# the3cloud/zktls

Measured on AMD Instinct MI355X. Metric: trace-cells/s, higher is better.
Workload: dtype u32

## Files before the change

zktls_amd/csrc/stark.hip:

```cpp
#include <atomic>

#include "poseidon2.cuh"
#include "kernels.h"
#include "batch.h"

namespace zk {

hipError_t stark_upload_p2_tables(const P2Tables& t, hipStream_t s) { return p2_upload_tables(t, s); }


ZK_D Ext ld_ext(const uint32_t* p) {
    uint4 v = *reinterpret_cast<const uint4*>(p);
    return Ext{{v.x, v.y, v.z, v.w}};
}
ZK_D void st_ext(uint32_t* p, const Ext& e) { *reinterpret_cast<uint4*>(p) = make_uint4(e.c[0], e.c[1], e.c[2], e.c[3]); }

ZK_D Ext group_sum(Ext v, int width) {
    for (int off = width >> 1; off > 0; off >>= 1) {
        Ext o;
        o.c[0] = __shfl_down(v.c[0], off, width);
        o.c[1] = __shfl_down(v.c[1], off, width);
        o.c[2] = __shfl_down(v.c[2], off, width);
        o.c[3] = __shfl_down(v.c[3], off, width);
        v = Ext{{dadd(v.c[0], o.c[0]), dadd(v.c[1], o.c[1]), dadd(v.c[2], o.c[2]), dadd(v.c[3], o.c[3])}};
// ... 36 lines not shown
ZK_D uint4 ld_stream(const uint32_t* p) {
    const u32x4_nt v = __builtin_nontemporal_load(reinterpret_cast<const u32x4_nt*>(p));
    return make_uint4(v.x, v.y, v.z, v.w);
}
ZK_D void dacc1(uint64_t& acc, uint32_t a0, uint32_t b0) {
    const uint64_t t = dmac(a0, b0, acc);
    acc = ((uint64_t)dred((uint32_t)(t >> 32)) << 32) | (uint32_t)t;
}
template <int CTRL>
ZK_D uint32_t dpp_mov(uint32_t v) { return (uint32_t)__builtin_amdgcn_update_dpp(0, (int)v, CTRL, 0xF, 0xF, false); }
ZK_D uint32_t row_group_sum(uint32_t v, int L) {
    if (L > 1) v = dadd(v, dpp_mov<0xB1>(v));
    if (L > 2) v = dadd(v, dpp_mov<0x4E>(v));
    if (L > 4) v = dadd(v, dpp_mov<0x141>(v));
    if (L > 8) v = dadd(v, dpp_mov<0x140>(v));
    return v;
}
__device__ __forceinline__ void logup_addend_kernel_body(const QuotientArgs& a) {
    const int H = a.log_n + 1;
    const uint32_t m = 1u << H;
    const uint32_t p = blockIdx.x * blockDim.x + threadIdx.x;
    if (p >= m) return;
    const uint32_t e = __brev(p) >> (32 - H);
    const uint32_t pn = __brev((e + 2) & (m - 1)) >> (32 - H);
    const uint32_t* row = a.lde + (uint64_t)p * a.ld;
    const uint32_t* prow = a.perm + (uint64_t)p * a.perm_ld;
    const uint32_t* pnrow = a.perm + (uint64_t)pn * a.perm_ld;
    const uint32_t* wl = a.alpha_pow + 16 * (a.width / 4);
    const uint32_t sel_trans = dsub(a.xs[p], a.wn_inv);
    Ext r = ext_zero(), sphi = ext_zero(), sphin = ext_zero();
    for (uint32_t q = 0; q < a.pairs; q++) {
        const uint4 vs = *reinterpret_cast<const uint4*>(row + 8 * q);
        const uint4 vr = *reinterpret_cast<const uint4*>(row + 8 * q + 4);
        const Ext ds = ext_add(ext_add_base(a.gamma, vs.x), ext_mul_base_dev(a.beta, vs.y));
        const Ext dr = ext_add(ext_add_base(a.gamma, vr.x), ext_mul_base_dev(a.beta, vr.y));
        const Ext phi = ld_ext(prow + 4 * q), phin = ld_ext(pnrow + 4 * q);
        const Ext c = ext_sub(ext_mul_dev(ext_mul_dev(phi, ds), dr), ext_sub(dr, ds));
        r = ext_add(r, ext_mul_dev(c, ld_ext(wl + 4 * q)));
        sphi = ext_add(sphi, phi);
        sphin = ext_add(sphin, phin);
    }
    const Ext S = ld_ext(prow + 4 * a.pairs), Sn = ld_ext(pnrow + 4 * a.pairs);
    const Ext F1 = ext_mul_base_dev(ld_ext(wl + 4 * a.pairs), a.sel_first[p]);
    const Ext F2 = ext_mul_base_dev(ld_ext(wl + 4 * (a.pairs + 1)), sel_trans);
    const Ext F3 = ext_mul_base_dev(ld_ext(wl + 4 * (a.pairs + 2)), a.sel_last[p]);
    r = ext_add(r, ext_mul_dev(F1, ext_sub(S, sphi)));
    r = ext_add(r, ext_mul_dev(F2, ext_sub(ext_sub(Sn, S), sphin)));
    r = ext_add(r, ext_mul_dev(F3, ext_sub(S, a.cumsum)));
    st_ext(a.addend_out + 4 * (uint64_t)p, r);
}
__global__ void __launch_bounds__(256) logup_addend_kernel(QuotientArgs a) { logup_addend_kernel_body(a); }
struct logup_addend_kernel_bargs { QuotientArgs a; static logup_addend_kernel_bargs make(QuotientArgs a) { return logup_addend_kernel_bargs{a}; } };
__global__ void __launch_bounds__(256) logup_addend_kernel_batch(const logup_addend_kernel_bargs* __restrict__ zk_arr) { const logup_addend_kernel_bargs& zk_b = zk_arr[blockIdx.z]; logup_addend_kernel_body(zk_b.a); }

hipError_t launch_logup_addend(const QuotientArgs& a, hipStream_t s) {
    const uint64_t m = 2ull << a.log_n;
    ZK_LAUNCH(logup_addend_kernel, logup_addend_kernel_batch, logup_addend_kernel_bargs, dim3((unsigned)((m + 255) / 256)), dim3(256), 0, s, a);
    return hipGetLastError();
}
constexpr int QCHAIN = 16;
template <int NG>
#ifndef QWPE
#define QWPE 2
#endif
__device__ __forceinline__ void quotient_kernel_body(const QuotientArgs& a) {
    const int L = a.lanes_per_row;
    const uint32_t gid = blockIdx.x * blockDim.x + threadIdx.x;
    const int lane = gid % L;
    const int H = a.log_n + 1;
    const uint32_t m = 1u << H;
    const uint32_t nchains = m / QCHAIN;
    const bool live = gid / L < nchains;
    const uint32_t chain = live ? gid / L : 0u;
    const uint32_t parity = chain & 1u;
    uint32_t e = 2u * ((chain >> 1) * QCHAIN) + parity;
    const uint32_t G = a.width / 4;
    const uint32_t inv_zh = parity ? a.inv_zh_odd : a.inv_zh_even;

    uint4 cur[NG], nxt[NG];
    uint32_t p = __brev(e) >> (32 - H);
#pragma unroll
    for (int t = 0; t < NG; t++) {
        const uint32_t g = lane + L * t;
        cur[t] = g < G ? *reinterpret_cast<const uint4*>(a.lde + (uint64_t)p * a.ld + 4 * g) : make_uint4(0, 0, 0, 0);
    }
    constexpr bool HOIST = NG <= 4;
    uint4 W[HOIST ? NG : 1][4];
    if (HOIST) {
#pragma unroll
        for (int t = 0; t < NG; t++) {
            const uint32_t g = lane + L * t;
            const uint4* wp = reinterpret_cast<const uint4*>(a.alpha_pow + 16 * (g < G ? g : 0u));
#pragma unroll
            for (int i = 0; i < 4; i++) W[HOIST ? t : 0][i] = wp[i];
        }
    }
    for (int step = 0; step < QCHAIN; step++) {
        const uint32_t en = (e + 2) & (m - 1);
        const uint32_t pn = __brev(en) >> (32 - H);
#pragma unroll
        for (int t = 0; t < NG; t++) {
            const uint32_t g = lane + L * t;
            nxt[t] = g < G ? ld_stream(a.lde + (uint64_t)pn * a.ld + 4 * g) : make_uint4(0, 0, 0, 0);
        }
        const uint32_t x = a.xs[p];
        const uint32_t sel_first = a.sel_first[p];
        const uint32_t sel_trans = dsub(x, a.wn_inv);
        uint64_t acc[4] = {0, 0, 0, 0};
#pragma unroll
        for (int t = 0; t < NG; t++) {
            const uint32_t g = lane + L * t;
            if (g < G) {
                const uint4 v = cur[t];
                const uint4* wp = reinterpret_cast<const uint4*>(a.alpha_pow + 16 * g);
                const uint4 w0 = HOIST ? W[HOIST ? t : 0][0] : wp[0], w1 = HOIST ? W[HOIST ? t : 0][1] : wp[1];
                const uint4 w2 = HOIST ? W[HOIST ? t : 0][2] : wp[2], kk = HOIST ? W[HOIST ? t : 0][3] : wp[3];
                const uint32_t aab = dmul(dmont_lazy(v.x, v.x), v.y);
                const uint32_t c1 = dsub(dsub(v.z, aab), kk.x);
                const uint32_t ab = dmul(v.x, v.y);
                const uint32_t c2 = dmul(dsub_lazy(dsub(dsub(nxt[t].w, ab), v.z), kk.y), sel_trans);
                const uint32_t c3 = dmul(dsub_lazy(v.w, kk.z), sel_first);
                dacc2(acc[0], w0.x, c1, w1.x, c2); dacc1(acc[0], w2.x, c3);
                dacc2(acc[1], w0.y, c1, w1.y, c2); dacc1(acc[1], w2.y, c3);
                dacc2(acc[2], w0.z, c1, w1.z, c2); dacc1(acc[2], w2.z, c3);
                dacc2(acc[3], w0.w, c1, w1.w, c2); dacc1(acc[3], w2.w, c3);
            }
        }
        Ext r = Ext{{dacc_finish(acc[0]), dacc_finish(acc[1]), dacc_finish(acc[2]), dacc_finish(acc[3])}};
        if (a.addend && lane == 0) r = ext_add(r, ld_ext(a.addend + 4 * (uint64_t)p));
#pragma unroll
        for (int i = 0; i < 4; i++) r.c[i] = row_group_sum(r.c[i], L);
        if (lane == 0 && live) {
            r = ext_mul_base_dev(r, inv_zh);
            st_ext(a.out + ((uint64_t)parity * (m >> 1) + (e >> 1)) * 4, r);
            if (a.lde_out) st_ext(a.lde_out + (uint64_t)p * a.lde_ld + 4u * parity, r);
        }
#pragma unroll
        for (int t = 0; t < NG; t++) cur[t] = nxt[t];
        e = en; p = pn;
    }
}
template <int NG>
#ifndef QWPE
#define QWPE 2
#endif
__global__ void __launch_bounds__(256) __attribute__((amdgpu_waves_per_eu(QWPE, QWPE))) quotient_kernel(QuotientArgs a) { quotient_kernel_body<NG>(a); }
struct quotient_kernel_bargs { QuotientArgs a; static quotient_kernel_bargs make(QuotientArgs a) { return quotient_kernel_bargs{a}; } };
template <int NG>
#ifndef QWPE
#define QWPE 2
#endif
__global__ void __launch_bounds__(256) __attribute__((amdgpu_waves_per_eu(QWPE, QWPE))) quotient_kernel_batch(const quotient_kernel_bargs* __restrict__ zk_arr) { const quotient_kernel_bargs& zk_b = zk_arr[blockIdx.z]; quotient_kernel_body<NG>(zk_b.a); }

hipError_t launch_quotient(const QuotientArgs& a, hipStream_t s) {
    const uint64_t m = 2ull << a.log_n;
    const uint64_t threads = (m / QCHAIN) * a.lanes_per_row;
    const uint32_t G = a.width / 4;
    const int ng = (int)((G + a.lanes_per_row - 1) / a.lanes_per_row);
    const dim3 grid((unsigned)((threads + 255) / 256)), block(256);
    switch (ng) {
        case 1: ZK_LAUNCH(quotient_kernel<1>, quotient_kernel_batch<1>, quotient_kernel_bargs, grid, block, 0, s, a); break;
        case 2: ZK_LAUNCH(quotient_kernel<2>, quotient_kernel_batch<2>, quotient_kernel_bargs, grid, block, 0, s, a); break;
        case 3: ZK_LAUNCH(quotient_kernel<3>, quotient_kernel_batch<3>, quotient_kernel_bargs, grid, block, 0, s, a); break;
        case 4: ZK_LAUNCH(quotient_kernel<4>, quotient_kernel_batch<4>, quotient_kernel_bargs, grid, block, 0, s, a); break;
        case 5: case 6: case 7: case 8: ZK_LAUNCH(quotient_kernel<8>, quotient_kernel_batch<8>, quotient_kernel_bargs, grid, block, 0, s, a); break;
        default: ZK_LAUNCH(quotient_kernel<16>, quotient_kernel_batch<16>, quotient_kernel_bargs, grid, block, 0, s, a); break;
    }
    return hipGetLastError();
}

__device__ __forceinline__ void quotient_air_kernel_body(const QuotientAirArgs& a) {
    const int H = a.log_n + a.log_qd;
    const uint32_t m = 1u << H, nq = 1u << a.log_qd;
    const uint32_t p = blockIdx.x * blockDim.x + threadIdx.x;
    if (p >= m) return;
    const uint32_t e = __brev(p) >> (32 - H);
    const uint32_t pn = __brev((e + nq) & (m - 1)) >> (32 - H);
    const uint32_t* local = a.lde + (uint64_t)p * a.ld;
    const uint32_t* next = a.lde + (uint64_t)pn * a.ld;
    const uint32_t x = a.xs[p];
    const uint32_t sel_first = a.sel_first[p], sel_last = a.sel_last[p], sel_trans = dsub(x, a.wn_inv);
    uint64_t acc[4] = {0, 0, 0, 0};
    const uint32_t* w = a.body;
    for (uint32_t k = 0; k < a.n_constraints; k++) {
        const uint32_t sel = *w++, nt = *w++;
        uint32_t c = 0;
        for (uint32_t t = 0; t < nt; t++) {
            uint32_t prod = *w++;
            const uint32_t d = *w++;
            for (uint32_t j = 0; j < d; j++) {
                const uint32_t v = *w++, kind = v >> 30, idx = v & 0xFFFFu;
                const uint32_t val = kind == 0 ? local[idx] : (kind == 1 ? next[idx] : a.pub[idx]);
                prod = dmul(prod, val);
            }
            c = dadd(c, prod);
        }
        if (sel) c = dmul(c, sel == 1 ? sel_first : (sel == 2 ? sel_last : sel_trans));
        const uint4 wt = *reinterpret_cast<const uint4*>(a.weights + 4 * (uint64_t)k);
        dacc1(acc[0], wt.x, c); dacc1(acc[1], wt.y, c); dacc1(acc[2], wt.z, c); dacc1(acc[3], wt.w, c);
    }
    const uint32_t chunk = e & (nq - 1u);
    Ext r = Ext{{dacc_finish(acc[0]), dacc_finish(acc[1]), dacc_finish(acc[2]), dacc_finish(acc[3])}};
    if (a.addend) r = ext_add(r, ld_ext(a.addend + 4 * (uint64_t)p));
    const uint32_t iz = chunk == 0 ? a.inv_zh[0] : (chunk == 1 ? a.inv_zh[1] : (chunk == 2 ? a.inv_zh[2] : a.inv_zh[3]));
    r = ext_mul_base_dev(r, iz);
    st_ext(a.out + ((uint64_t)chunk * (m >> a.log_qd) + (e >> a.log_qd)) * 4, r);
    if (a.lde_out) st_ext(a.lde_out + (uint64_t)p * a.lde_ld + 4u * chunk, r);
}
__global__ void __launch_bounds__(256) quotient_air_kernel(QuotientAirArgs a) { quotient_air_kernel_body(a); }
struct quotient_air_kernel_bargs { QuotientAirArgs a; static quotient_air_kernel_bargs make(QuotientAirArgs a) { return quotient_air_kernel_bargs{a}; } };
__global__ void __launch_bounds__(256) quotient_air_kernel_batch(const quotient_air_kernel_bargs* __restrict__ zk_arr) { const quotient_air_kernel_bargs& zk_b = zk_arr[blockIdx.z]; quotient_air_kernel_body(zk_b.a); }

__device__ __forceinline__ uint32_t air_group_e0(const QuotientAirArgs& a, uint32_t g) { return ((g >> a.log_qd) * 8u << a.log_qd) + (g & ((1u << a.log_qd) - 1u)); }
__device__ __forceinline__ uint32_t air_row_of(const QuotientAirArgs& a, uint32_t e0, uint32_t r) {
    const int H = a.log_n + a.log_qd;
    return __brev((e0 + (r << a.log_qd)) & ((1u << H) - 1u)) >> (32 - H);
}
__device__ __forceinline__ void air_load8(const uint32_t* slots, uint32_t base, uint32_t (&v)[8]) {
    const uint32_t* b = slots + base;
#pragma unroll
    for (int q = 0; q < 8; q++) v[q] = b[4 * q];
}
template <int NT>
__device__ __forceinline__ void air_stage_extras(const QuotientAirArgs& a, uint32_t* slots, uint32_t e0, uint32_t tid) {
    const uint32_t W4 = a.width >> 2;
    if (tid < 8) {
        const uint32_t p = air_row_of(a, e0, tid);
        const uint4 ex = {a.sel_first[p], a.sel_last[p], dsub(a.xs[p], a.wn_inv), MONTY_R1};
        *reinterpret_cast<uint4*>(slots + AIR_GP * W4 + 4u * tid) = ex;
    }
    for (uint32_t i = tid >> 3; i < a.n_public; i += NT / 8) slots[air_lds_base(2 * a.width + AIR_SLOT_EXTRA + i, a.width) + 4u * (tid & 7u)] = a.pub[i];
}
__device__ __forceinline__ void air_store_point(const QuotientAirArgs& a, uint32_t e, Ext r) {
    const int H = a.log_n + a.log_qd;
    const uint32_t m = 1u << H, nq = 1u << a.log_qd;
    const uint32_t p = __brev(e) >> (32 - H);
    if (a.addend) r = ext_add(r, ld_ext(a.addend + 4 * (uint64_t)p));
    const uint32_t chunk = e & (nq - 1u);
    const uint32_t iz = chunk == 0 ? a.inv_zh[0] : (chunk == 1 ? a.inv_zh[1] : (chunk == 2 ? a.inv_zh[2] : a.inv_zh[3]));
    r = ext_mul_base_dev(r, iz);
    st_ext(a.out + ((uint64_t)chunk * (m >> a.log_qd) + (e >> a.log_qd)) * 4, r);
    if (a.lde_out) st_ext(a.lde_out + (uint64_t)p * a.lde_ld + 4u * chunk, r);
}
template <int NT>
__device__ __forceinline__ void quotient_air_terms_kernel_body(const QuotientAirArgs& a) {
    constexpr int PTS = 8;
    static_assert(NT == 64 || NT == 128 || NT == 256, "one, two or four wavefronts per group");
    extern __shared__ uint32_t slots[];
    const uint32_t tid = threadIdx.x, W4 = a.width >> 2;
    const uint32_t mask = (1u << (a.log_n + a.log_qd)) - 1u;
    const uint32_t e0 = air_group_e0(a, blockIdx.x);
#pragma unroll
    for (int r = 0; r < 9; r++) {
        const uint4* row = reinterpret_cast<const uint4*>(a.lde + (uint64_t)air_row_of(a, e0, r) * a.ld);
        for (uint32_t cg = tid; cg < W4; cg += NT) *reinterpret_cast<uint4*>(slots + AIR_GP * cg + 4u * r) = row[cg];
    }
    air_stage_extras<NT>(a, slots, e0, tid);
    __syncthreads();
    uint64_t acc[PTS][4];
#pragma unroll
    for (int q = 0; q < PTS; q++)
#pragma unroll
        for (int i = 0; i < 4; i++) acc[q][i] = 0;
    const uint4* recs = reinterpret_cast<const uint4*>(a.recs);
    auto load8 = [&](uint32_t o, uint32_t (&v)[PTS]) { air_load8(slots, o, v); };
    auto product = [&](const uint4& o, uint32_t (&prod)[PTS]) {
        const uint32_t n = o.z >> 16;
        uint32_t v[PTS];
        load8(o.x & 0xFFFFu, prod);
        const uint32_t offs[4] = {o.x >> 16, o.y & 0xFFFFu, o.y >> 16, o.z & 0xFFFFu};
        for (uint32_t k = 1; k < n; k++) {
            load8(offs[k - 1], v);
#pragma unroll
            for (int q = 0; q < PTS; q++) prod[q] = dmul(prod[q], v[q]);
        }
    };
    for (uint32_t t = 2 * tid; t < a.n_terms; t += 2 * NT) {
        const uint4 ca = recs[2 * (size_t)t], oa = recs[2 * (size_t)t + 1], cb = recs[2 * (size_t)t + 2], ob = recs[2 * (size_t)t + 3];
        uint32_t pa[PTS], pb[PTS];
        product(oa, pa);
        product(ob, pb);
#pragma unroll
        for (int q = 0; q < PTS; q++) {
            dacc2(acc[q][0], ca.x, pa[q], cb.x, pb[q]); dacc2(acc[q][1], ca.y, pa[q], cb.y, pb[q]);
            dacc2(acc[q][2], ca.z, pa[q], cb.z, pb[q]); dacc2(acc[q][3], ca.w, pa[q], cb.w, pb[q]);
        }
    }
    __syncthreads();
    constexpr int PITCH = NT + 1, SL = NT / 32;
#pragma unroll
    for (int q = 0; q < PTS; q++)
#pragma unroll
        for (int i = 0; i < 4; i++) slots[(size_t)(q * 4 + i) * PITCH + tid] = dacc_finish(acc[q][i]);
    __syncthreads();
    {
        const uint32_t j = tid / SL, sl = tid % SL;
        uint32_t sum = 0;
        for (uint32_t i = sl; i < (uint32_t)NT; i += SL) sum = dadd(sum, slots[(size_t)j * PITCH + i]);
        __syncthreads();
        slots[(size_t)j * PITCH + sl] = sum;
    }
    __syncthreads();
    if (tid < (uint32_t)PTS) {
        Ext r;
        for (int i = 0; i < 4; i++) {
            uint32_t sum = 0;
            for (int k = 0; k < SL; k++) sum = dadd(sum, slots[(size_t)(tid * 4 + i) * PITCH + k]);
            r.c[i] = sum;
// ... 473 lines not shown
        }
#pragma unroll
        for (int k = 0; k < NPTS; k++) {
            Ext w[4];
#pragma unroll
            for (int j = 0; j < 4; j++) w[j] = ld_ext(a.xw + 4 * ((uint64_t)k * a.xw_stride + q[j]));
#pragma unroll
            for (int i = 0; i < 4; i++) {
                dacc2(acc[k][i][0], v[0].x, w[0].c[i], v[1].x, w[1].c[i]); dacc2(acc[k][i][0], v[2].x, w[2].c[i], v[3].x, w[3].c[i]);
                dacc2(acc[k][i][1], v[0].y, w[0].c[i], v[1].y, w[1].c[i]); dacc2(acc[k][i][1], v[2].y, w[2].c[i], v[3].y, w[3].c[i]);
                dacc2(acc[k][i][2], v[0].z, w[0].c[i], v[1].z, w[1].c[i]); dacc2(acc[k][i][2], v[2].z, w[2].c[i], v[3].z, w[3].c[i]);
                dacc2(acc[k][i][3], v[0].w, w[0].c[i], v[1].w, w[1].c[i]); dacc2(acc[k][i][3], v[2].w, w[2].c[i], v[3].w, w[3].c[i]);
            }
        }
    }
#pragma unroll
    for (int k = 0; k < NPTS; k++) {
        uint32_t mine[16];
#pragma unroll
        for (int c = 0; c < 4; c++)
#pragma unroll
            for (int i = 0; i < 4; i++) mine[4 * c + i] = dacc_finish(acc[k][i][c]);
        __syncthreads();
#pragma unroll
        for (int e = 0; e < 16; e++) red[threadIdx.x * 16 + e] = mine[e];
        __syncthreads();
        if (ty == 0 && active) {
            for (int y = 1; y < TY; y++)
#pragma unroll
                for (int e = 0; e < 16; e++) mine[e] = dadd(mine[e], red[(y * TX + tx) * 16 + e]);
            uint4* dst = reinterpret_cast<uint4*>(a.partial + 4 * (((uint64_t)blockIdx.x * NPTS + k) * a.width + col));
#pragma unroll
            for (int c = 0; c < 4; c++) dst[c] = make_uint4(mine[4 * c], mine[4 * c + 1], mine[4 * c + 2], mine[4 * c + 3]);
        }
    }
}
template <int NPTS>
__global__ void __launch_bounds__(256) open_partial4_kernel(OpenArgs a) { open_partial4_kernel_body<NPTS>(a); }
struct open_partial4_kernel_bargs { OpenArgs a; static open_partial4_kernel_bargs make(OpenArgs a) { return open_partial4_kernel_bargs{a}; } };
template <int NPTS>
__global__ void __launch_bounds__(256) open_partial4_kernel_batch(const open_partial4_kernel_bargs* __restrict__ zk_arr) { const open_partial4_kernel_bargs& zk_b = zk_arr[blockIdx.z]; open_partial4_kernel_body<NPTS>(zk_b.a); }

__device__ __forceinline__ void open_final_kernel_body(const uint32_t* partial, uint32_t nchunks, int npts, uint32_t width, const Ext& scale0, const Ext& scale1, uint32_t* out) {
    const uint32_t idx = blockIdx.x;
    const uint32_t k = idx / width, col = idx % width;
    Ext sum = ext_zero();
    for (uint32_t c = threadIdx.x; c < nchunks; c += 64) sum = ext_add(sum, ld_ext(partial + 4 * (((uint64_t)c * npts + k) * width + col)));
    sum = group_sum(sum, 64);
    if (threadIdx.x == 0) st_ext(out + 4 * (uint64_t)idx, ext_neg(ext_mul_dev(sum, k ? scale1 : scale0)));
}
__global__ void __launch_bounds__(64) open_final_kernel(const uint32_t* partial, uint32_t nchunks, int npts, uint32_t width, Ext scale0, Ext scale1, uint32_t* out) { open_final_kernel_body(partial, nchunks, npts, width, scale0, scale1, out); }
struct open_final_kernel_bargs { const uint32_t* partial; uint32_t nchunks; int npts; uint32_t width; Ext scale0; Ext scale1; uint32_t* out; static open_final_kernel_bargs make(const uint32_t* partial, uint32_t nchunks, int npts, uint32_t width, Ext scale0, Ext scale1, uint32_t* out) { return open_final_kernel_bargs{partial, nchunks, npts, width, scale0, scale1, out}; } };
__global__ void __launch_bounds__(64) open_final_kernel_batch(const open_final_kernel_bargs* __restrict__ zk_arr) { const open_final_kernel_bargs& zk_b = zk_arr[blockIdx.z]; open_final_kernel_body(zk_b.partial, zk_b.nchunks, zk_b.npts, zk_b.width, zk_b.scale0, zk_b.scale1, zk_b.out); }

bool open_uses_quads(uint32_t width, uint64_t ld, const uint32_t* mat) {
    return width >= 64 && width % 4 == 0 && ld % 4 == 0 && ((uintptr_t)mat & 15u) == 0;
}
size_t open_chunks(uint64_t rows, uint32_t width, uint64_t ld, const uint32_t* mat) {
    const uint64_t per = open_uses_quads(width, ld, mat) ? OPEN_ROWS4 : OPEN_ROWS;
    return (size_t)((rows + per - 1) / per);
}
hipError_t launch_open(const OpenArgs& a0, int npts, const Ext& scale0, const Ext& scale1, uint32_t* out, hipStream_t s) {
    OpenArgs a = a0;
    const bool quads = open_uses_quads(a.width, a.ld, a.mat);
    const uint32_t nchunks = (uint32_t)open_chunks(a.rows, a.width, a.ld, a.mat);
    if (quads) {
        a.tx = 1;
        while (a.tx < (int)(a.width / 4) && a.tx < 64) a.tx <<= 1;
        dim3 grid(nchunks, (a.width / 4 + a.tx - 1) / a.tx);
        if (npts == 1) ZK_LAUNCH(open_partial4_kernel<1>, open_partial4_kernel_batch<1>, open_partial4_kernel_bargs, grid, dim3(256), 0, s, a);
        else ZK_LAUNCH(open_partial4_kernel<2>, open_partial4_kernel_batch<2>, open_partial4_kernel_bargs, grid, dim3(256), 0, s, a);
    } else {
        dim3 grid(nchunks, (a.width + a.tx - 1) / a.tx);
        if (npts == 1) ZK_LAUNCH(open_partial_kernel<1>, open_partial_kernel_batch<1>, open_partial_kernel_bargs, grid, dim3(256), 0, s, a);
        else ZK_LAUNCH(open_partial_kernel<2>, open_partial_kernel_batch<2>, open_partial_kernel_bargs, grid, dim3(256), 0, s, a);
    }
    hipError_t e = hipGetLastError();
    if (e != hipSuccess) return e;
    const uint32_t n = (uint32_t)npts * a.width;
    ZK_LAUNCH(open_final_kernel, open_final_kernel_batch, open_final_kernel_bargs, dim3(n), dim3(64), 0, s, a.partial, nchunks, npts, a.width, scale0, scale1, out);
    return hipGetLastError();
}

__device__ __forceinline__ void rowdot_kernel_body(const uint32_t* __restrict__ mat, uint64_t ld, uint32_t width, uint64_t rows, int L, const uint32_t* __restrict__ alpha_pow, uint32_t* __restrict__ out_at) {
    const uint64_t gid = (uint64_t)blockIdx.x * blockDim.x + threadIdx.x;
    const uint64_t p = gid / L;
    const int lane = (int)(gid % L);
    if (p >= rows) return;
    const uint32_t* row = mat + p * ld;
    uint64_t acc[4] = {0, 0, 0, 0};
    const uint32_t nq = width / 4;
    for (uint32_t q = lane; q < nq; q += L) {
        const uint4 v = ld_stream(row + 4 * q);
        const uint4* ap = reinterpret_cast<const uint4*>(alpha_pow + 16 * q);
        const uint4 a0 = ap[0], a1 = ap[1], a2 = ap[2], a3 = ap[3];
        dacc2(acc[0], a0.x, v.x, a1.x, v.y); dacc2(acc[0], a2.x, v.z, a3.x, v.w);
        dacc2(acc[1], a0.y, v.x, a1.y, v.y); dacc2(acc[1], a2.y, v.z, a3.y, v.w);
        dacc2(acc[2], a0.z, v.x, a1.z, v.y); dacc2(acc[2], a2.z, v.z, a3.z, v.w);
        dacc2(acc[3], a0.w, v.x, a1.w, v.y); dacc2(acc[3], a2.w, v.z, a3.w, v.w);
    }
    Ext r;
#pragma unroll
    for (int i = 0; i < 4; i++) r.c[i] = row_group_sum(dacc_finish(acc[i]), L);
    if (lane == 0) st_ext(out_at + 4 * p, r);
}
__global__ void __launch_bounds__(256) rowdot_kernel(const uint32_t* __restrict__ mat, uint64_t ld, uint32_t width, uint64_t rows, int L, const uint32_t* __restrict__ alpha_pow, uint32_t* __restrict__ out_at) { rowdot_kernel_body(mat, ld, width, rows, L, alpha_pow, out_at); }
struct rowdot_kernel_bargs { const uint32_t* mat; uint64_t ld; uint32_t width; uint64_t rows; int L; const uint32_t* alpha_pow; uint32_t* out_at; static rowdot_kernel_bargs make(const uint32_t* mat, uint64_t ld, uint32_t width, uint64_t rows, int L, const uint32_t* alpha_pow, uint32_t* out_at) { return rowdot_kernel_bargs{mat, ld, width, rows, L, alpha_pow, out_at}; } };
__global__ void __launch_bounds__(256) rowdot_kernel_batch(const rowdot_kernel_bargs* __restrict__ zk_arr) { const rowdot_kernel_bargs& zk_b = zk_arr[blockIdx.z]; rowdot_kernel_body(zk_b.mat, zk_b.ld, zk_b.width, zk_b.rows, zk_b.L, zk_b.alpha_pow, zk_b.out_at); }

constexpr int ROWDOT_TRIPS = 16;
template <int NK>
__device__ __forceinline__ void rowdot_regs_kernel_body(const uint32_t* __restrict__ mat, uint64_t ld, uint32_t width, uint64_t rows, int L, const uint32_t* __restrict__ alpha_pow, uint32_t* __restrict__ out_at) {
    const int lane = (int)(threadIdx.x % L);
    const uint32_t nq = width / 4;
    const uint64_t rows_per_trip = 256 / L;
    const uint64_t r0 = (uint64_t)blockIdx.x * rows_per_trip * ROWDOT_TRIPS + threadIdx.x / L;
    uint4 a0[NK], a1[NK], a2[NK], a3[NK];
#pragma unroll
    for (int k = 0; k < NK; k++) {
        const uint32_t q = lane + (uint32_t)L * k;
        const uint4* ap = reinterpret_cast<const uint4*>(alpha_pow + 16 * (q < nq ? q : 0));
        a0[k] = ap[0]; a1[k] = ap[1]; a2[k] = ap[2]; a3[k] = ap[3];
    }
    for (int t = 0; t < ROWDOT_TRIPS; t++) {
        const uint64_t p = r0 + (uint64_t)t * rows_per_trip;
        if (p >= rows) return;
        const uint32_t* row = mat + p * ld;
        uint4 v[NK];
#pragma unroll
        for (int k = 0; k < NK; k++) {
            const uint32_t q = lane + (uint32_t)L * k;
            v[k] = q < nq ? ld_stream(row + 4 * q) : make_uint4(0, 0, 0, 0);
        }
        uint64_t acc[4] = {0, 0, 0, 0};
#pragma unroll
        for (int k = 0; k < NK; k++) {
            dacc2(acc[0], a0[k].x, v[k].x, a1[k].x, v[k].y); dacc2(acc[0], a2[k].x, v[k].z, a3[k].x, v[k].w);
            dacc2(acc[1], a0[k].y, v[k].x, a1[k].y, v[k].y); dacc2(acc[1], a2[k].y, v[k].z, a3[k].y, v[k].w);
            dacc2(acc[2], a0[k].z, v[k].x, a1[k].z, v[k].y); dacc2(acc[2], a2[k].z, v[k].z, a3[k].z, v[k].w);
            dacc2(acc[3], a0[k].w, v[k].x, a1[k].w, v[k].y); dacc2(acc[3], a2[k].w, v[k].z, a3[k].w, v[k].w);
        }
        Ext r;
#pragma unroll
        for (int i = 0; i < 4; i++) r.c[i] = row_group_sum(dacc_finish(acc[i]), L);
        if (lane == 0) st_ext(out_at + 4 * p, r);
    }
}
template <int NK>
__global__ void __launch_bounds__(256) rowdot_regs_kernel(const uint32_t* __restrict__ mat, uint64_t ld, uint32_t width, uint64_t rows, int L, const uint32_t* __restrict__ alpha_pow, uint32_t* __restrict__ out_at) { rowdot_regs_kernel_body<NK>(mat, ld, width, rows, L, alpha_pow, out_at); }
struct rowdot_regs_kernel_bargs { const uint32_t* mat; uint64_t ld; uint32_t width; uint64_t rows; int L; const uint32_t* alpha_pow; uint32_t* out_at; static rowdot_regs_kernel_bargs make(const uint32_t* mat, uint64_t ld, uint32_t width, uint64_t rows, int L, const uint32_t* alpha_pow, uint32_t* out_at) { return rowdot_regs_kernel_bargs{mat, ld, width, rows, L, alpha_pow, out_at}; } };
template <int NK>
__global__ void __launch_bounds__(256) rowdot_regs_kernel_batch(const rowdot_regs_kernel_bargs* __restrict__ zk_arr) { const rowdot_regs_kernel_bargs& zk_b = zk_arr[blockIdx.z]; rowdot_regs_kernel_body<NK>(zk_b.mat, zk_b.ld, zk_b.width, zk_b.rows, zk_b.L, zk_b.alpha_pow, zk_b.out_at); }

static hipError_t launch_rowdot(const uint32_t* mat, uint64_t ld, uint32_t width, uint64_t rows, const uint32_t* alpha_pow, uint32_t* out_at, hipStream_t s);
__device__ __forceinline__ void reduced_combine_kernel_body(const ReducedArgs& a, const uint32_t* __restrict__ at_in, const uint32_t* __restrict__ ap_in) {
    const uint64_t p = (uint64_t)blockIdx.x * blockDim.x + threadIdx.x;
    if (p >= a.rows) return;
    const Ext at = ld_ext(at_in + 4 * p);
    const uint4* qrow = reinterpret_cast<const uint4*>(a.qlde + p * a.q_ld);
    Ext aq = ext_zero();
    for (uint32_t h = 0; h < a.q_width / 8; h++) {
        const uint4 q0 = qrow[2 * h], q1 = qrow[2 * h + 1];
        const uint32_t qv[8] = {q0.x, q0.y, q0.z, q0.w, q1.x, q1.y, q1.z, q1.w};
#pragma unroll
        for (int j = 0; j < 8; j++) aq = ext_add(aq, ext_mul_base_dev(ld_ext(a.alpha_pow + 4 * (8 * h + j)), qv[j]));
    }
    const Ext d1 = ld_ext(a.dinv + 4 * p), d2 = ld_ext(a.dinv + 4 * (a.rows + p));
    Ext r = ext_mul_dev(a.off_loc, ext_mul_dev(ext_sub(at, a.y_loc), d1));
    r = ext_add(r, ext_mul_dev(a.off_next, ext_mul_dev(ext_sub(at, a.y_next), d2)));
    if (a.p_width) {
        const Ext ap = ld_ext(ap_in + 4 * p);
        r = ext_add(r, ext_mul_dev(a.off_pl, ext_mul_dev(ext_sub(ap, a.y_pl), d1)));
        r = ext_add(r, ext_mul_dev(a.off_pn, ext_mul_dev(ext_sub(ap, a.y_pn), d2)));
    }
    r = ext_add(r, ext_mul_dev(a.off_q, ext_mul_dev(ext_sub(aq, a.y_q), d1)));
    if (a.accumulate) r = ext_add(r, ld_ext(a.out + 4 * p));
    st_ext(a.out + 4 * p, r);
}
__global__ void __launch_bounds__(256) reduced_combine_kernel(ReducedArgs a, const uint32_t* __restrict__ at_in, const uint32_t* __restrict__ ap_in) { reduced_combine_kernel_body(a, at_in, ap_in); }
struct reduced_combine_kernel_bargs { ReducedArgs a; const uint32_t* at_in; const uint32_t* ap_in; static reduced_combine_kernel_bargs make(ReducedArgs a, const uint32_t* at_in, const uint32_t* ap_in) { return reduced_combine_kernel_bargs{a, at_in, ap_in}; } };
__global__ void __launch_bounds__(256) reduced_combine_kernel_batch(const reduced_combine_kernel_bargs* __restrict__ zk_arr) { const reduced_combine_kernel_bargs& zk_b = zk_arr[blockIdx.z]; reduced_combine_kernel_body(zk_b.a, zk_b.at_in, zk_b.ap_in); }

static int lanes_for(uint32_t width) { int g = (int)(width / 4), l = 1; while (l < g && l < 16) l <<= 1; return l; }
int rowdot_form(uint32_t width, uint64_t rows) {
    const int L = lanes_for(width);
    const uint32_t nq = width / 4;
    const int nk = (int)((nq + L - 1) / L);
    const uint64_t rows_per_wg = (uint64_t)(256 / L) * ROWDOT_TRIPS;
    return (nk >= 1 && nk <= 4 && rows % (256 / L) == 0 && rows >= rows_per_wg) ? nk : 0;
}
static hipError_t launch_rowdot(const uint32_t* mat, uint64_t ld, uint32_t width, uint64_t rows, const uint32_t* alpha_pow, uint32_t* out_at, hipStream_t s) {
    const int L = lanes_for(width);
    const int form = rowdot_form(width, rows);
    if (form) {
        const uint64_t rows_per_wg = (uint64_t)(256 / L) * ROWDOT_TRIPS;
        const dim3 grid((unsigned)((rows + rows_per_wg - 1) / rows_per_wg)), block(256);
        switch (form) {
            case 1: ZK_LAUNCH(rowdot_regs_kernel<1>, rowdot_regs_kernel_batch<1>, rowdot_regs_kernel_bargs, grid, block, 0, s, mat, ld, width, rows, L, alpha_pow, out_at); break;
            case 2: ZK_LAUNCH(rowdot_regs_kernel<2>, rowdot_regs_kernel_batch<2>, rowdot_regs_kernel_bargs, grid, block, 0, s, mat, ld, width, rows, L, alpha_pow, out_at); break;
            case 3: ZK_LAUNCH(rowdot_regs_kernel<3>, rowdot_regs_kernel_batch<3>, rowdot_regs_kernel_bargs, grid, block, 0, s, mat, ld, width, rows, L, alpha_pow, out_at); break;
            default: ZK_LAUNCH(rowdot_regs_kernel<4>, rowdot_regs_kernel_batch<4>, rowdot_regs_kernel_bargs, grid, block, 0, s, mat, ld, width, rows, L, alpha_pow, out_at); break;
        }
        return hipGetLastError();
    }
    const uint64_t threads = rows * L;
    ZK_LAUNCH(rowdot_kernel, rowdot_kernel_batch, rowdot_kernel_bargs, dim3((unsigned)((threads + 255) / 256)), dim3(256), 0, s, mat, ld, width, rows, L, alpha_pow, out_at);
    return hipGetLastError();
}
hipError_t launch_reduced_opening(const ReducedArgs& a, uint32_t* scratch_at, hipStream_t s) {
    hipError_t e = launch_rowdot(a.tlde, a.t_ld, a.width, a.rows, a.alpha_pow, scratch_at, s);
    if (e != hipSuccess) return e;
    uint32_t* scratch_ap = scratch_at + 4 * a.rows;
    if (a.p_width) {
        e = launch_rowdot(a.plde, a.p_ld, a.p_width, a.rows, a.alpha_pow, scratch_ap, s);
        if (e != hipSuccess) return e;
    }
    ZK_LAUNCH(reduced_combine_kernel, reduced_combine_kernel_batch, reduced_combine_kernel_bargs, dim3((unsigned)((a.rows + 255) / 256)), dim3(256), 0, s, a, scratch_at, scratch_ap);
    return hipGetLastError();
}

constexpr int PERM_BLOCK = 256;
__device__ __forceinline__ void perm_rows_kernel_body(const PermArgs& a, uint32_t* __restrict__ block_tot) {
    __shared__ uint32_t sh[PERM_BLOCK * 4];
    const uint64_t i = (uint64_t)blockIdx.x * PERM_BLOCK + threadIdx.x;
    Ext sum = ext_zero();
    if (i < a.rows) {
        const uint32_t* row = a.trace + i * a.ld;
        uint32_t* prow = a.out + i * a.out_ld;
        for (uint32_t q = 0; q < a.pairs; q++) {
            const uint4 vs = *reinterpret_cast<const uint4*>(row + 8 * q);
            const uint4 vr = *reinterpret_cast<const uint4*>(row + 8 * q + 4);
            const Ext ds = ext_add(ext_add_base(a.gamma, vs.x), ext_mul_base_dev(a.beta, vs.y));
            const Ext dr = ext_add(ext_add_base(a.gamma, vr.x), ext_mul_base_dev(a.beta, vr.y));
            const Ext d = ext_mul_dev(ds, dr);
            const Ext phi = ext_eq(d, ext_zero()) ? ext_sub(ext_inv_dev(ds), ext_inv_dev(dr)) : ext_mul_dev(ext_sub(dr, ds), ext_inv_dev(d));
            st_ext(prow + 4 * q, phi);
            sum = ext_add(sum, phi);
        }
    }
    for (int k = 0; k < 4; k++) sh[threadIdx.x * 4 + k] = sum.c[k];
    __syncthreads();
    for (int off = 1; off < PERM_BLOCK; off <<= 1) {
        Ext o = ext_zero();
        if ((int)threadIdx.x >= off) o = Ext{{sh[(threadIdx.x - off) * 4], sh[(threadIdx.x - off) * 4 + 1], sh[(threadIdx.x - off) * 4 + 2], sh[(threadIdx.x - off) * 4 + 3]}};
        __syncthreads();
        sum = ext_add(sum, o);
        for (int k = 0; k < 4; k++) sh[threadIdx.x * 4 + k] = sum.c[k];
        __syncthreads();
    }
    if (i < a.rows) st_ext(a.out + i * a.out_ld + 4 * a.pairs, sum);
    if (threadIdx.x == PERM_BLOCK - 1) st_ext(block_tot + 4 * (uint64_t)blockIdx.x, sum);
}
__global__ void __launch_bounds__(PERM_BLOCK) perm_rows_kernel(PermArgs a, uint32_t* __restrict__ block_tot) { perm_rows_kernel_body(a, block_tot); }
struct perm_rows_kernel_bargs { PermArgs a; uint32_t* block_tot; static perm_rows_kernel_bargs make(PermArgs a, uint32_t* block_tot) { return perm_rows_kernel_bargs{a, block_tot}; } };
__global__ void __launch_bounds__(PERM_BLOCK) perm_rows_kernel_batch(const perm_rows_kernel_bargs* __restrict__ zk_arr) { const perm_rows_kernel_bargs& zk_b = zk_arr[blockIdx.z]; perm_rows_kernel_body(zk_b.a, zk_b.block_tot); }

__device__ __forceinline__ void perm_scan_blocks_kernel_body(uint32_t* block_tot, uint32_t nblocks) {
    __shared__ uint32_t sh[1024 * 4];
    const uint32_t per = (nblocks + 1023) / 1024;
    const uint32_t b0 = threadIdx.x * per;
    Ext sum = ext_zero();
    for (uint32_t k = 0; k < per && b0 + k < nblocks; k++) sum = ext_add(sum, ld_ext(block_tot + 4 * (uint64_t)(b0 + k)));
    for (int k = 0; k < 4; k++) sh[threadIdx.x * 4 + k] = sum.c[k];
    __syncthreads();
    Ext incl = sum;
    for (int off = 1; off < 1024; off <<= 1) {
        Ext o = ext_zero();
        if ((int)threadIdx.x >= off) o = Ext{{sh[(threadIdx.x - off) * 4], sh[(threadIdx.x - off) * 4 + 1], sh[(threadIdx.x - off) * 4 + 2], sh[(threadIdx.x - off) * 4 + 3]}};
        __syncthreads();
        incl = ext_add(incl, o);
        for (int k = 0; k < 4; k++) sh[threadIdx.x * 4 + k] = incl.c[k];
        __syncthreads();
    }
    Ext run = ext_sub(incl, sum);
    for (uint32_t k = 0; k < per && b0 + k < nblocks; k++) {
        const Ext t = ld_ext(block_tot + 4 * (uint64_t)(b0 + k));
        st_ext(block_tot + 4 * (uint64_t)(b0 + k), run);
        run = ext_add(run, t);
    }
}
__global__ void __launch_bounds__(1024) perm_scan_blocks_kernel(uint32_t* block_tot, uint32_t nblocks) { perm_scan_blocks_kernel_body(block_tot, nblocks); }
struct perm_scan_blocks_kernel_bargs { uint32_t* block_tot; uint32_t nblocks; static perm_scan_blocks_kernel_bargs make(uint32_t* block_tot, uint32_t nblocks) { return perm_scan_blocks_kernel_bargs{block_tot, nblocks}; } };
__global__ void __launch_bounds__(1024) perm_scan_blocks_kernel_batch(const perm_scan_blocks_kernel_bargs* __restrict__ zk_arr) { const perm_scan_blocks_kernel_bargs& zk_b = zk_arr[blockIdx.z]; perm_scan_blocks_kernel_body(zk_b.block_tot, zk_b.nblocks); }

__device__ __forceinline__ void perm_fixup_kernel_body(const PermArgs& a, const uint32_t* __restrict__ block_off) {
    const uint64_t i = (uint64_t)blockIdx.x * PERM_BLOCK + threadIdx.x;
    if (i >= a.rows) return;
    uint32_t* sp = a.out + i * a.out_ld + 4 * a.pairs;
    st_ext(sp, ext_add(ld_ext(sp), ld_ext(block_off + 4 * (uint64_t)blockIdx.x)));
}
__global__ void __launch_bounds__(PERM_BLOCK) perm_fixup_kernel(PermArgs a, const uint32_t* __restrict__ block_off) { perm_fixup_kernel_body(a, block_off); }
struct perm_fixup_kernel_bargs { PermArgs a; const uint32_t* block_off; static perm_fixup_kernel_bargs make(PermArgs a, const uint32_t* block_off) { return perm_fixup_kernel_bargs{a, block_off}; } };
__global__ void __launch_bounds__(PERM_BLOCK) perm_fixup_kernel_batch(const perm_fixup_kernel_bargs* __restrict__ zk_arr) { const perm_fixup_kernel_bargs& zk_b = zk_arr[blockIdx.z]; perm_fixup_kernel_body(zk_b.a, zk_b.block_off); }

hipError_t launch_perm_trace(const PermArgs& a, uint32_t* block_scratch, hipStream_t s) {
    const uint32_t nblocks = (uint32_t)((a.rows + PERM_BLOCK - 1) / PERM_BLOCK);
    ZK_LAUNCH(perm_rows_kernel, perm_rows_kernel_batch, perm_rows_kernel_bargs, dim3(nblocks), dim3(PERM_BLOCK), 0, s, a, block_scratch);
    hipError_t e = hipGetLastError();
    if (e != hipSuccess) return e;
    ZK_LAUNCH(perm_scan_blocks_kernel, perm_scan_blocks_kernel_batch, perm_scan_blocks_kernel_bargs, dim3(1), dim3(1024), 0, s, block_scratch, nblocks);
    e = hipGetLastError();
    if (e != hipSuccess) return e;
    ZK_LAUNCH(perm_fixup_kernel, perm_fixup_kernel_batch, perm_fixup_kernel_bargs, dim3(nblocks), dim3(PERM_BLOCK), 0, s, a, block_scratch);
    return hipGetLastError();
}

ZK_D Ext lookup_fingerprint(const LookupArgs& lk, const uint32_t* rec, const uint32_t* row, const uint8_t* cm = nullptr) {
    Ext d = ext_add_base(lk.gamma, rec[2]);
    for (uint32_t v = 0; v < rec[3]; v++) d = ext_add(d, ext_mul_base_dev(lk.bpow[v + 1], row[cm ? cm[rec[4 + v]] : rec[4 + v]]));
    return d;
}
ZK_D uint32_t lookup_mult(const uint32_t* rec, const uint32_t* row, const uint8_t* cm = nullptr) {
    const uint32_t m = rec[1] == 0xFFFFFFFFu ? MONTY_R1 : row[cm ? cm[rec[1]] : rec[1]];
    return rec[0] ? (m ? P - m : 0u) : m;
}
ZK_D const uint32_t* lookup_stage_rows(const LookupArgs& lk, const uint32_t* mat, uint64_t ld, uint64_t row0, uint64_t rows, uint32_t* dyn, const uint8_t** cm_out,
                                       const uint32_t* pre = nullptr, uint64_t pre_ld = 0, uint32_t pre_w = 0) {
    uint8_t* cm = reinterpret_cast<uint8_t*>(dyn);
    uint32_t* tile = dyn + LOOKUP_MAX_COLS / 4;
    const uint32_t pitch = lk.n_used | 1u, tid = threadIdx.x;
    for (uint32_t i = tid; i < LOOKUP_MAX_COLS / 4; i += blockDim.x) dyn[i] = reinterpret_cast<const uint32_t*>(lk.cmap)[i];
    __syncthreads();
    const uint32_t q = tid & 3u;
    for (uint32_t m = lk.chunk_mask; m; m &= m - 1u) {
        const uint32_t col = 16u * (uint32_t)(__ffs((int)m) - 1) + 4u * q;
        const uint8_t k0 = cm[col], k1 = cm[col + 1], k2 = cm[col + 2], k3 = cm[col + 3];
        if ((k0 & k1 & k2 & k3) == 0xFF) continue;
        for (uint32_t r = tid >> 2; r < 256u; r += blockDim.x >> 2) {
            if (row0 + r >= rows) break;
            const bool from_pre = pre != nullptr && col < pre_w;
            const uint32_t* src = from_pre ? pre + (row0 + r) * pre_ld + col : mat + (row0 + r) * ld + (col - (pre ? pre_w : 0u));
            uint32_t* dst = tile + r * pitch;
            if (from_pre || col - (pre ? pre_w : 0u) + 3 < ld) {
                const uint4 v = *reinterpret_cast<const uint4*>(src);
                if (k0 != 0xFF) dst[k0] = v.x;
                if (k1 != 0xFF) dst[k1] = v.y;
                if (k2 != 0xFF) dst[k2] = v.z;
                if (k3 != 0xFF) dst[k3] = v.w;
            } else {
                const uint32_t mc = col - (pre ? pre_w : 0u);
                if (k0 != 0xFF && mc < ld) dst[k0] = src[0];
                if (k1 != 0xFF && mc + 1 < ld) dst[k1] = src[1];
                if (k2 != 0xFF && mc + 2 < ld) dst[k2] = src[2];
            }
        }
    }
// ... 213 lines not shown
```

Baseline: 20.95 billion.

## Add LDS-staged streaming kernels for quotient and row-dot reductions

Adds new quotient and rowdot kernels in which each wave stages 64 rows × 32 columns slices through a padded LDS tile. Loads are coalesced and the next slice is prefetched into registers, so each lane reduces one full row with no cross-lane shuffle reduction. The quotient path also reads the neighbouring row from LDS for the transition constraint. This is meant to cut uncoalesced strided global loads and shuffle overhead, at the cost of LDS use and wave-level fences, and only applies when the width is a multiple of 32 and there are enough rows.

Result: faster. 21.36 billion (median of 6 runs) (+2.0%).

```diff
diff --git a/zktls_amd/csrc/stark.hip b/zktls_amd/csrc/stark.hip
--- a/zktls_amd/csrc/stark.hip
+++ b/zktls_amd/csrc/stark.hip
@@ -212,8 +212,100 @@
 #endif
 __global__ void __launch_bounds__(256) __attribute__((amdgpu_waves_per_eu(QWPE, QWPE))) quotient_kernel_batch(const quotient_kernel_bargs* __restrict__ zk_arr) { const quotient_kernel_bargs& zk_b = zk_arr[blockIdx.z]; quotient_kernel_body<NG>(zk_b.a); }
 
+constexpr int SLICE_COLS = 32;
+constexpr int SLICE_PITCH = SLICE_COLS + 4;
+constexpr uint64_t STREAM_MIN_ROWS = 2048;
+ZK_D void wave_lds_handover() {
+    __builtin_amdgcn_fence(__ATOMIC_RELEASE, "wavefront");
+    __builtin_amdgcn_wave_barrier();
+    __builtin_amdgcn_fence(__ATOMIC_ACQUIRE, "wavefront");
+}
+#ifdef ZKHIP_AB_HOOKS
+static bool stream_forms_off() { const char* e = getenv("ZKHIP_STREAM_OLD"); return e && atoi(e) != 0; }
+#endif
+
+__device__ __forceinline__ void quotient_stream_kernel_body(const QuotientArgs& a) {
+    __shared__ __attribute__((aligned(16))) uint32_t tile[4][65 * SLICE_PITCH];
+    const uint32_t lane = threadIdx.x & 63u, wave = threadIdx.x >> 6;
+    const int H = a.log_n + 1;
+    const uint32_t m = 1u << H;
+    const uint32_t wpp = m >> 7;
+    const uint32_t gw = blockIdx.x * 4u + wave;
+    if (gw >= 2u * wpp) return;
+    const uint32_t parity = gw / wpp, j0 = (gw % wpp) * 64u;
+    uint32_t* t = tile[wave];
+    const uint32_t part = lane & 7u, sub = lane >> 3;
+    const uint32_t* src[9];
+#pragma unroll
+    for (int k = 0; k < 9; k++) {
+        const uint32_t j = j0 + 8u * k + (k < 8 ? sub : 0u);
+        const uint32_t pr = __brev((2u * j + parity) & (m - 1)) >> (32 - H);
+        src[k] = a.lde + (uint64_t)pr * a.ld + 4u * part;
+    }
+    const bool tail = lane < 8u;
+    uint4 pf[9];
+#pragma unroll
+    for (int k = 0; k < 8; k++) pf[k] = ld_stream(src[k]);
+    pf[8] = tail ? ld_stream(src[8]) : make_uint4(0, 0, 0, 0);
+
+    const uint32_t j = j0 + lane;
+    const uint32_t p = __brev(2u * j + parity) >> (32 - H);
+    uint32_t sel_first = a.sel_first[p];
+    const uint32_t sel_trans = dsub(a.xs[p], a.wn_inv);
+    asm("" : "+v"(sel_first));
+    const uint32_t nsl = a.width / SLICE_COLS;
+    uint64_t acc[4] = {0, 0, 0, 0};
+    for (uint32_t s = 0; s < nsl; s++) {
+#pragma unroll
+        for (int k = 0; k < 8; k++) *reinterpret_cast<uint4*>(t + (8u * k + sub) * SLICE_PITCH + 4u * part) = pf[k];
+        if (tail) *reinterpret_cast<uint4*>(t + 64u * SLICE_PITCH + 4u * part) = pf[8];
+        if (s + 1 < nsl) {
+#pragma unroll
+            for (int k = 0; k < 8; k++) pf[k] = ld_stream(src[k] + SLICE_COLS * (s + 1));
+            if (tail) pf[8] = ld_stream(src[8] + SLICE_COLS * (s + 1));
+        }
+        wave_lds_handover();
+        const uint4* wp = reinterpret_cast<const uint4*>(a.alpha_pow + 16u * (SLICE_COLS / 4) * s);
+#pragma unroll
+        for (int g = 0; g < SLICE_COLS / 4; g++) {
+            const uint4 v = *reinterpret_cast<const uint4*>(t + lane * SLICE_PITCH + 4 * g);
+            const uint32_t dn = t[(lane + 1u) * SLICE_PITCH + 4 * g + 3];
+            const uint4 w0 = wp[4 * g], w1 = wp[4 * g + 1], w2 = wp[4 * g + 2], kk = wp[4 * g + 3];
+            const uint32_t aab = dmul(dmont_lazy(v.x, v.x), v.y);
+            const uint32_t c1 = dsub(dsub(v.z, aab), kk.x);
+            const uint32_t ab = dmul(v.x, v.y);
+            const uint32_t c2 = dmul(dsub_lazy(dsub(dsub(dn, ab), v.z), kk.y), sel_trans);
+            const uint32_t c3 = dmul(dsub_lazy(v.w, kk.z), sel_first);
+            dacc2(acc[0], w0.x, c1, w1.x, c2); dacc1(acc[0], w2.x, c3);
+            dacc2(acc[1], w0.y, c1, w1.y, c2); dacc1(acc[1], w2.y, c3);
+            dacc2(acc[2], w0.z, c1, w1.z, c2); dacc1(acc[2], w2.z, c3);
+            dacc2(acc[3], w0.w, c1, w1.w, c2); dacc1(acc[3], w2.w, c3);
+        }
+        wave_lds_handover();
+    }
+    Ext r = Ext{{dacc_finish(acc[0]), dacc_finish(acc[1]), dacc_finish(acc[2]), dacc_finish(acc[3])}};
+    if (a.addend) r = ext_add(r, ld_ext(a.addend + 4 * (uint64_t)p));
+    r = ext_mul_base_dev(r, parity ? a.inv_zh_odd : a.inv_zh_even);
+    st_ext(a.out + ((uint64_t)parity * (m >> 1) + j) * 4, r);
+    if (a.lde_out) st_ext(a.lde_out + (uint64_t)p * a.lde_ld + 4u * parity, r);
+}
+__global__ void __launch_bounds__(256) quotient_stream_kernel(QuotientArgs a) { quotient_stream_kernel_body(a); }
+struct quotient_stream_kernel_bargs { QuotientArgs a; static quotient_stream_kernel_bargs make(QuotientArgs a) { return quotient_stream_kernel_bargs{a}; } };
+__global__ void __launch_bounds__(256) quotient_stream_kernel_batch(const quotient_stream_kernel_bargs* __restrict__ zk_arr) { const quotient_stream_kernel_bargs& zk_b = zk_arr[blockIdx.z]; quotient_stream_kernel_body(zk_b.a); }
+
+static bool quotient_stream_form(const QuotientArgs& a) {
+#ifdef ZKHIP_AB_HOOKS
+    if (stream_forms_off()) return false;
+#endif
+    return a.width % SLICE_COLS == 0 && (2ull << a.log_n) >= STREAM_MIN_ROWS;
+}
+
 hipError_t launch_quotient(const QuotientArgs& a, hipStream_t s) {
     const uint64_t m = 2ull << a.log_n;
+    if (quotient_stream_form(a)) {
+        ZK_LAUNCH(quotient_stream_kernel, quotient_stream_kernel_batch, quotient_stream_kernel_bargs, dim3((unsigned)(m / 256)), dim3(256), 0, s, a);
+        return hipGetLastError();
+    }
     const uint64_t threads = (m / QCHAIN) * a.lanes_per_row;
     const uint32_t G = a.width / 4;
     const int ng = (int)((G + a.lanes_per_row - 1) / a.lanes_per_row);
@@ -993,6 +1085,45 @@
 template <int NK>
 __global__ void __launch_bounds__(256) rowdot_regs_kernel_batch(const rowdot_regs_kernel_bargs* __restrict__ zk_arr) { const rowdot_regs_kernel_bargs& zk_b = zk_arr[blockIdx.z]; rowdot_regs_kernel_body<NK>(zk_b.mat, zk_b.ld, zk_b.width, zk_b.rows, zk_b.L, zk_b.alpha_pow, zk_b.out_at); }
 
+__device__ __forceinline__ void rowdot_stream_kernel_body(const uint32_t* __restrict__ mat, uint64_t ld, uint32_t width, uint64_t rows, const uint32_t* __restrict__ alpha_pow, uint32_t* __restrict__ out_at) {
+    __shared__ __attribute__((aligned(16))) uint32_t tile[4][64 * SLICE_PITCH];
+    const uint32_t lane = threadIdx.x & 63u, wave = threadIdx.x >> 6;
+    const uint64_t r0 = ((uint64_t)blockIdx.x * 4u + wave) * 64u;
+    if (r0 >= rows) return;
+    uint32_t* t = tile[wave];
+    const uint32_t part = lane & 7u, sub = lane >> 3;
+    const uint32_t* src = mat + (r0 + sub) * ld + 4u * part;
+    uint4 pf[8];
+#pragma unroll
+    for (int k = 0; k < 8; k++) pf[k] = ld_stream(src + 8u * k * ld);
+    const uint32_t nsl = width / SLICE_COLS;
+    uint64_t acc[4] = {0, 0, 0, 0};
+    for (uint32_t s = 0; s < nsl; s++) {
+#pragma unroll
+        for (int k = 0; k < 8; k++) *reinterpret_cast<uint4*>(t + (8u * k + sub) * SLICE_PITCH + 4u * part) = pf[k];
+        if (s + 1 < nsl) {
+#pragma unroll
+            for (int k = 0; k < 8; k++) pf[k] = ld_stream(src + 8u * k * ld + SLICE_COLS * (s + 1));
+        }
+        wave_lds_handover();
+        const uint4* ap = reinterpret_cast<const uint4*>(alpha_pow + 16u * (SLICE_COLS / 4) * s);
+#pragma unroll
+        for (int q = 0; q < SLICE_COLS / 4; q++) {
+            const uint4 v = *reinterpret_cast<const uint4*>(t + lane * SLICE_PITCH + 4 * q);
+            const uint4 a0 = ap[4 * q], a1 = ap[4 * q + 1], a2 = ap[4 * q + 2], a3 = ap[4 * q + 3];
+            dacc2(acc[0], a0.x, v.x, a1.x, v.y); dacc2(acc[0], a2.x, v.z, a3.x, v.w);
+            dacc2(acc[1], a0.y, v.x, a1.y, v.y); dacc2(acc[1], a2.y, v.z, a3.y, v.w);
+            dacc2(acc[2], a0.z, v.x, a1.z, v.y); dacc2(acc[2], a2.z, v.z, a3.z, v.w);
+            dacc2(acc[3], a0.w, v.x, a1.w, v.y); dacc2(acc[3], a2.w, v.z, a3.w, v.w);
+        }
+        wave_lds_handover();
+    }
+    st_ext(out_at + 4 * (r0 + lane), Ext{{dacc_finish(acc[0]), dacc_finish(acc[1]), dacc_finish(acc[2]), dacc_finish(acc[3])}});
+}
+__global__ void __launch_bounds__(256) rowdot_stream_kernel(const uint32_t* __restrict__ mat, uint64_t ld, uint32_t width, uint64_t rows, const uint32_t* __restrict__ alpha_pow, uint32_t* __restrict__ out_at) { rowdot_stream_kernel_body(mat, ld, width, rows, alpha_pow, out_at); }
+struct rowdot_stream_kernel_bargs { const uint32_t* mat; uint64_t ld; uint32_t width; uint64_t rows; const uint32_t* alpha_pow; uint32_t* out_at; static rowdot_stream_kernel_bargs make(const uint32_t* mat, uint64_t ld, uint32_t width, uint64_t rows, const uint32_t* alpha_pow, uint32_t* out_at) { return rowdot_stream_kernel_bargs{mat, ld, width, rows, alpha_pow, out_at}; } };
+__global__ void __launch_bounds__(256) rowdot_stream_kernel_batch(const rowdot_stream_kernel_bargs* __restrict__ zk_arr) { const rowdot_stream_kernel_bargs& zk_b = zk_arr[blockIdx.z]; rowdot_stream_kernel_body(zk_b.mat, zk_b.ld, zk_b.width, zk_b.rows, zk_b.alpha_pow, zk_b.out_at); }
+
 static hipError_t launch_rowdot(const uint32_t* mat, uint64_t ld, uint32_t width, uint64_t rows, const uint32_t* alpha_pow, uint32_t* out_at, hipStream_t s);
 __device__ __forceinline__ void reduced_combine_kernel_body(const ReducedArgs& a, const uint32_t* __restrict__ at_in, const uint32_t* __restrict__ ap_in) {
     const uint64_t p = (uint64_t)blockIdx.x * blockDim.x + threadIdx.x;
@@ -1033,6 +1164,14 @@
 static hipError_t launch_rowdot(const uint32_t* mat, uint64_t ld, uint32_t width, uint64_t rows, const uint32_t* alpha_pow, uint32_t* out_at, hipStream_t s) {
     const int L = lanes_for(width);
     const int form = rowdot_form(width, rows);
+    bool stream = form && width % SLICE_COLS == 0 && rows % 64 == 0 && rows >= STREAM_MIN_ROWS;
+#ifdef ZKHIP_AB_HOOKS
+    if (stream_forms_off()) stream = false;
+#endif
+    if (stream) {
+        ZK_LAUNCH(rowdot_stream_kernel, rowdot_stream_kernel_batch, rowdot_stream_kernel_bargs, dim3((unsigned)((rows + 255) / 256)), dim3(256), 0, s, mat, ld, width, rows, alpha_pow, out_at);
+        return hipGetLastError();
+    }
     if (form) {
         const uint64_t rows_per_wg = (uint64_t)(256 / L) * ROWDOT_TRIPS;
         const dim3 grid((unsigned)((rows + rows_per_wg - 1) / rows_per_wg)), block(256);
```
